# peleiden/librubiks

Hardware: AMD Instinct MI355X
Metric: cube node-expansions/sec (12-child fan-out) at 1M-state batch (higher is better)
Workload: dtype u8

## Files before the change

librubiks_amd/csrc/rk_cube_kernels.hip:

```cpp
#include <algorithm>
#include <atomic>
#include <cstdlib>
#include <mutex>
#include <vector>

#include "rk_device.h"
#include "rk_kernels.h"

namespace rk {

constexpr int EXP_ROUND = 64;
constexpr int EXP_WAVES = 4;
constexpr unsigned PACE_TAU_PS = 2100;
constexpr unsigned PACE_ROT_TAU_PS = 1200;
constexpr unsigned PACE_SOLVED_TAU_PS = 0;
constexpr unsigned PACE_LEAD_TICKS = 50;
constexpr unsigned PACE_PULL_WGS = 128;
constexpr unsigned PACE_PULL_WGS_FIRST = 256;
constexpr unsigned PACE_PHASE_TILES = 16384;
constexpr size_t PACE_MIN_TILES = 3072;
constexpr unsigned PACE686_MIN_PARENTS = 65536;
constexpr unsigned long long PACE_MAX_WAIT_TICKS = 2000;
constexpr unsigned long long PACE_STALE_TICKS = 1500;
constexpr size_t PACE_FIRST_TILES = 16384;
// ... 612 lines not shown
			#pragma unroll
			for (int k = 0; k < 20; k++) {
				const int idx = k * 64 + lane;
				buf_dw[idx] = idx < ndw ? got[k] : 0xFFFFFFFFu;
			}
		}
		wave_lds_fence();
		u32x4 v[5];
		#pragma unroll
		for (int k = 0; k < 5; k++) v[k] = buf[lane * 5 + k];
		const uint32_t s[20] = {v[0].x, v[0].y, v[0].z, v[0].w, v[1].x, v[1].y, v[1].z, v[1].w, v[2].x, v[2].y, v[2].z, v[2].w,
		                        v[3].x, v[3].y, v[3].z, v[3].w, v[4].x, v[4].y, v[4].z, v[4].w};
		uint32_t fl = 0;
		#pragma unroll
		for (int q = 0; q < 4; q++)
			if (4 * lane + q < np && is_solved5(&s[5 * q])) fl |= 1u << (8 * q);
		if (flags != nullptr) {
			uint8_t *fdst = flags + p0;
			if (np == ROW_TILE && ((reinterpret_cast<uintptr_t>(fdst) & 3) == 0)) {
				reinterpret_cast<uint32_t *>(fdst)[lane] = fl;
			} else {
				#pragma unroll
				for (int q = 0; q < 4; q++)
					if (4 * lane + q < np) fdst[4 * lane + q] = (uint8_t)((fl >> (8 * q)) & 1u);
			}
		}
		if (stats != nullptr && __ballot(fl != 0u) != 0ull && fl != 0u) {
			atomicAdd(reinterpret_cast<unsigned long long *>(&stats[0]), (unsigned long long)__popc(fl));
			const int firstq = (__ffs(fl) - 1) >> 3;
			atomicMin(&stats[1], (long long)(p0 + 4 * lane + firstq));
		}
		wave_lds_fence();
	}
}

template <int CH>
__device__ __forceinline__ void fetch_actions(const uint8_t *__restrict__ actions, size_t games, size_t g, int d0, int todo, uint32_t (&a)[CH])
{
	#pragma unroll
	for (int k = 0; k < CH; k++) a[k] = d0 + k < todo ? (uint32_t)actions[(size_t)(d0 + k) * games + g] : 0xFFu;
}

__global__ __launch_bounds__(256)
void k_apply_sequences(const uint8_t *__restrict__ actions, int moves, int games, int with_solved, int only_last,
                       uint32_t *__restrict__ out)
{
	__shared__ u32x4 s_act[36];
	stage_action_tables(s_act, threadIdx.x);
	__syncthreads();
	const int g = blockIdx.x * blockDim.x + threadIdx.x;
	if (g >= games) return;
	uint32_t s[5] = {SOLVED_DW[0], SOLVED_DW[1], SOLVED_DW[2], SOLVED_DW[3], SOLVED_DW[4]};
	const int rows = moves + (with_solved ? 1 : 0);
	uint32_t *o = out + (size_t)g * (only_last ? 1 : rows) * STATE_DWORDS;
	if (!only_last && with_solved) {
		#pragma unroll
		for (int j = 0; j < 5; j++) o[j] = s[j];
		o += STATE_DWORDS;
	}
	uint32_t worst = 0;
	constexpr int CH = 16;
	for (int d0 = 0; d0 < moves; d0 += CH) {
		uint32_t acts[CH];
		fetch_actions<CH>(actions, (size_t)games, (size_t)g, d0, moves, acts);
		#pragma unroll
		for (int k = 0; k < CH; k++) {
			if (d0 + k < moves) {
				uint32_t a = acts[k];
				worst = a > worst ? a : worst;
				a = a < 12u ? a : 0u;
				uint32_t tab[12];
				load_action_table(s_act, a, tab);
				move5(s, tab);
				if (!only_last) {
					#pragma unroll
					for (int j = 0; j < 5; j++) o[j] = s[j];
					o += STATE_DWORDS;
				}
			}
		}
	}
	if (only_last) {
		#pragma unroll
		for (int j = 0; j < 5; j++) o[j] = s[j];
	}
	if (worst >= 12u) atomicOr(&g_bad_actions, 1u);
}

__device__ __forceinline__ void scan_moves(uint32_t (&X)[12], int lane, int seg, int len)
{
	for (int off = 1; off < len; off <<= 1) {
		uint32_t Y[12];
		const int src = (lane - off) & 63;
		#pragma unroll
		for (int j = 0; j < 12; j++) Y[j] = (uint32_t)__builtin_amdgcn_ds_bpermute(src << 2, (int)X[j]);
		if (seg >= off) {
			uint32_t Z[12];
			#pragma unroll
			for (int j = 0; j < 6; j++) { Z[j] = lut4(Y[j], X); Z[6 + j] = lut4(Y[6 + j], X + 6); }
			#pragma unroll
			for (int j = 0; j < 12; j++) X[j] = Z[j];
		}
	}
}
__device__ __forceinline__ void identity_moves(uint32_t (&X)[12])
{
	#pragma unroll
	for (int j = 0; j < 6; j++) X[j] = X[6 + j] = 0x03020100u + 0x04040404u * (uint32_t)j;
}

__global__ __launch_bounds__(256)
void k_apply_sequences_scan(const uint8_t *__restrict__ actions, int moves, int games, int with_solved, int only_last, uint32_t *__restrict__ out)
{
	__shared__ u32x4 s_act[36];
	stage_action_tables(s_act, threadIdx.x);
	__syncthreads();
	const int lane = threadIdx.x & 63, g = blockIdx.x * 4 + (threadIdx.x >> 6);
	if (g >= games) return;
	uint32_t s[5] = {SOLVED_DW[0], SOLVED_DW[1], SOLVED_DW[2], SOLVED_DW[3], SOLVED_DW[4]};
	const int rows = moves + (with_solved ? 1 : 0);
	uint32_t *o = out + (size_t)g * (only_last ? 1 : rows) * STATE_DWORDS;
	if (!only_last && with_solved) {
		if (lane < 5) o[lane] = SOLVED_DW[lane];
		o += STATE_DWORDS;
	}
	uint32_t worst = 0;
	uint32_t a_next = lane < moves ? (uint32_t)actions[(size_t)lane * games + g] : 0xFFu;
	for (int d0 = 0; d0 < moves; d0 += 64) {
		const int n = moves - d0 < 64 ? moves - d0 : 64;
		uint32_t a = a_next;
		a_next = d0 + 64 + lane < moves ? (uint32_t)actions[(size_t)(d0 + 64 + lane) * games + g] : 0xFFu;
		uint32_t X[12];
		if (lane < n) {
			worst = a > worst ? a : worst;
			a = a < 12u ? a : 0u;
			load_action_table(s_act, a, X);
		} else {
			identity_moves(X);
		}
		scan_moves(X, lane, lane, n);
		uint32_t st[5] = {s[0], s[1], s[2], s[3], s[4]};
		move5(st, X);
		if (!only_last && lane < n) {
			#pragma unroll
			for (int j = 0; j < 5; j++) o[(size_t)(d0 + lane) * STATE_DWORDS + j] = st[j];
		}
		#pragma unroll
		for (int j = 0; j < 5; j++) s[j] = (uint32_t)__builtin_amdgcn_readlane((int)st[j], n - 1);
	}
	if (only_last && lane < 5) o[lane] = s[lane];
	if (worst >= 12u) atomicOr(&g_bad_actions, 1u);
}

__global__ __launch_bounds__(EXP_WAVES * WAVE)
void k_rollout_fanout(const uint8_t *__restrict__ actions, int moves, int games, int with_solved, uint32_t *__restrict__ states,
                      uint8_t *__restrict__ state_flags, u32x4 *__restrict__ children, uint32_t *__restrict__ solved, long long *__restrict__ stats)
{
	__shared__ u32x4 s_act[36];
	__shared__ u32x4 s_rows[48];
	__shared__ ExpandWaveLdsT<1> s_wave[EXP_WAVES];
	const int tid = threadIdx.x, lane = tid & 63, wv = tid >> 6;
	stage_action_tables(s_act, tid);
	if (tid < 48) {
		const uint32_t *src = reinterpret_cast<const uint32_t *>(D_TAB.rows) + 4 * tid;
		s_rows[tid] = u32x4{src[0], src[1], src[2], src[3]};
	}
	__syncthreads();
	const int rows = moves + (with_solved ? 1 : 0);
	const size_t n = (size_t)games * rows;
	const bool scan = rows <= EXP_ROUND;
	const int tile_states = scan ? (EXP_ROUND / rows) * rows : EXP_ROUND;
	const size_t p0 = ((size_t)blockIdx.x * EXP_WAVES + wv) * tile_states;
	if (p0 >= n) return;
	const int np = n - p0 < (size_t)tile_states ? (int)(n - p0) : tile_states;
	const size_t me = p0 + (lane < np ? lane : np - 1);
	const int g = (int)(me / rows), r = (int)(me - (size_t)g * rows);
	uint32_t par[5] = {SOLVED_DW[0], SOLVED_DW[1], SOLVED_DW[2], SOLVED_DW[3], SOLVED_DW[4]};
	uint32_t worst = 0;
	if (scan) {
		uint32_t X[12];
		const int mv = with_solved ? r - 1 : r;
		if (mv >= 0) {
			uint32_t a = actions[(size_t)mv * games + g];
			worst = a;
			a = a < 12u ? a : 0u;
			load_action_table(s_act, a, X);
		} else {
			identity_moves(X);
		}
		scan_moves(X, lane, r, rows);
		move5(par, X);
	} else {
		const int todo = with_solved ? r : r + 1;
		constexpr int CH = 16;
		for (int d0 = 0; d0 < todo; d0 += CH) {
			uint32_t acts[CH];
			fetch_actions<CH>(actions, (size_t)games, (size_t)g, d0, todo, acts);
			#pragma unroll
			for (int k = 0; k < CH; k++) {
				if (d0 + k < todo) {
					uint32_t a = acts[k];
					worst = a > worst ? a : worst;
					a = a < 12u ? a : 0u;
					uint32_t tab[12];
					load_action_table(s_act, a, tab);
					move5(par, tab);
				}
			}
		}
	}
	if (worst >= 12u) atomicOr(&g_bad_actions, 1u);
	const ExpandCtx c{s_rows, s_wave[wv].stage, s_wave[wv].flags, lane};
	uint32_t *stage_dw = reinterpret_cast<uint32_t *>(c.stage);
	#pragma unroll
	for (int j = 0; j < 5; j++) stage_dw[lane * 5 + j] = par[j];
	wave_lds_fence();
	#pragma unroll
	for (int k = 0; k < 5; k++) {
		const int idx = k * 64 + lane;
		if (idx < np * STATE_DWORDS) states[p0 * STATE_DWORDS + idx] = stage_dw[idx];
	}
	if (state_flags != nullptr && lane < np) state_flags[p0 + lane] = is_solved5(par) ? 1 : 0;
	wave_lds_fence();
	uint32_t out[60], fl[3];
	expand_lane<true>(c, par, out, fl);
	c.flags[lane * 3 + 0] = fl[0];
	c.flags[lane * 3 + 1] = fl[1];
	c.flags[lane * 3 + 2] = fl[2];
	#pragma unroll
	for (int v = 0; v < 15; v++)
		c.stage[lane * 15 + v] = u32x4{out[4 * v], out[4 * v + 1], out[4 * v + 2], out[4 * v + 3]};
	wave_lds_fence();
	u32x4 *dst = children + p0 * 15;
	const int nvec = np * 15;
	#pragma unroll
	for (int v = 0; v < 15; v++) {
		const int idx = v * 64 + lane;
		if (idx < nvec) store16<1>(dst, idx, c.stage[idx]);
	}
	uint32_t *fdst = solved + p0 * 3;
	#pragma unroll
	for (int k = 0; k < 3; k++) {
		const int idx = k * 64 + lane;
		if (idx < np * 3) fdst[idx] = c.flags[idx];
	}
	report_solved<true>(fl, lane < np, (p0 + lane) * 12, stats);
}

template <typename T> struct OhOne;
template <> struct OhOne<float>    { static constexpr uint32_t bits = 0x3F800000u; };
template <> struct OhOne<_Float16> { static constexpr uint32_t bits = 0x3C00u; };
struct bf16_tag {};
template <> struct OhOne<bf16_tag> { static constexpr uint32_t bits = 0x3F80u; };

template <typename T, int ELEM_BYTES, int TILE = 64, bool NT = false, int THREADS = 256>
__global__ __launch_bounds__(THREADS)
void k_as_oh(const uint32_t *__restrict__ states, u32x4 *__restrict__ out, size_t n, size_t n_tiles, unsigned tau_ps = 0, unsigned lead = 0,
             unsigned pull_wgs = 0, unsigned phase_tiles = 0, unsigned long long *pace = nullptr)
{
	constexpr int E = 16 / ELEM_BYTES;
	constexpr int CHUNKS_PER_ROW = 480 / E;
	constexpr int CHUNKS_PER_CUBIE = 24 / E;
	__shared__ uint32_t s_st[TILE * STATE_DWORDS];
	const int tid = threadIdx.x;
	const uint8_t *s_bytes = reinterpret_cast<const uint8_t *>(s_st);
	unsigned long long start = 0, base = 0;
	size_t tile_first = blockIdx.x, tile_stride = gridDim.x, slot = 0;
	if (tau_ps > 0) {
		const unsigned wgs_per_phase = pull_wgs + phase_tiles;
		const unsigned phase = blockIdx.x / wgs_per_phase, r = blockIdx.x - phase * wgs_per_phase;
		if (r < pull_wgs) {
			const size_t p_first = (size_t)phase * phase_tiles * TILE;
			const size_t p_count = n - p_first < (size_t)phase_tiles * TILE ? n - p_first : (size_t)phase_tiles * TILE;
			pull_front(states + p_first * STATE_DWORDS, p_count, (size_t)r * (THREADS / 64) + (tid >> 6), (size_t)pull_wgs * (THREADS / 64), tid & 63);
			if (tid == 0 && ((r & 63) == 63 || r + 1 == pull_wgs))
				__hip_atomic_fetch_max(pace, (unsigned long long)__builtin_amdgcn_s_memrealtime(), __ATOMIC_RELAXED, __HIP_MEMORY_SCOPE_AGENT);
			return;
		}
		start = __builtin_amdgcn_s_memrealtime();
		slot = r - pull_wgs;
		tile_first = (size_t)phase * phase_tiles + slot;
		tile_stride = n_tiles;
		if (pull_wgs == 0 && slot == 0 && tid == 0) __hip_atomic_fetch_max(pace, start, __ATOMIC_RELAXED, __HIP_MEMORY_SCOPE_AGENT);
		base = __hip_atomic_load(pace, __ATOMIC_RELAXED, __HIP_MEMORY_SCOPE_AGENT);
	}

	for (size_t tile = tile_first; tile < n_tiles; tile += tile_stride) {
		const size_t p0 = tile * TILE;
		const int np = (int)((n - p0 < (size_t)TILE) ? (n - p0) : (size_t)TILE);
		const int ndw = np * STATE_DWORDS;
		for (int idx = tid; idx < TILE * STATE_DWORDS; idx += THREADS) s_st[idx] = idx < ndw ? states[p0 * STATE_DWORDS + idx] : 0u;
		__syncthreads();
		PaceHold{base, start, slot, tau_ps, lead, tid & 63, pace}();
		const int nchunks = np * CHUNKS_PER_ROW;
		u32x4 *dst = out + p0 * CHUNKS_PER_ROW;
		for (int c = tid; c < nchunks; c += THREADS) {
			const int r = c / CHUNKS_PER_ROW, g = c - r * CHUNKS_PER_ROW;
			const int cubie = g / CHUNKS_PER_CUBIE;
			const int base = (g - cubie * CHUNKS_PER_CUBIE) * E;
			const int rel = (int)s_bytes[r * STATE_BYTES + cubie] - base;
			u32x4 val = {0u, 0u, 0u, 0u};
			if (ELEM_BYTES == 4) {
				val.x = rel == 0 ? OhOne<T>::bits : 0u;
				val.y = rel == 1 ? OhOne<T>::bits : 0u;
				val.z = rel == 2 ? OhOne<T>::bits : 0u;
				val.w = rel == 3 ? OhOne<T>::bits : 0u;
			} else {
				const uint32_t one = OhOne<T>::bits << (16 * (rel & 1));
				val.x = (rel >> 1) == 0 && rel >= 0 ? one : 0u;
				val.y = (rel >> 1) == 1 ? one : 0u;
				val.z = (rel >> 1) == 2 ? one : 0u;
				val.w = (rel >> 1) == 3 ? one : 0u;
			}
			if (NT) __builtin_nontemporal_store(val, dst + c);
			else dst[c] = val;
		}
		__syncthreads();
	}
}

__device__ __forceinline__ void stage_perm686(uint8_t *lds, int tid, int nthreads)
{
	const uint8_t *src = &D_TAB.perm686[0][0];
	for (int i = tid; i < N_ACTIONS * S686_SLOTS; i += nthreads) lds[i] = src[i];
}

template <bool FANOUT, bool FLAGS = false>
__global__ __launch_bounds__(256)
void k_rotate686(const uint16_t *__restrict__ states, const uint8_t *__restrict__ actions, u32x4 *__restrict__ out, size_t n_in,
                 uint8_t *__restrict__ flags = nullptr, long long *__restrict__ stats = nullptr)
{
	constexpr int GROUP = FANOUT ? 4 : 64;
	constexpr int OUT_PER_IN = FANOUT ? 12 : 1;
	__shared__ __attribute__((aligned(16))) uint8_t s_src[N_ACTIONS * 144];
	__shared__ __attribute__((aligned(16))) uint16_t s_in[GROUP * 144];
	__shared__ __attribute__((aligned(16))) uint8_t s_near[FLAGS ? N_ACTIONS * S686_SLOTS : 16];
	__shared__ __attribute__((aligned(16))) uint8_t s_col[FLAGS ? GROUP * S686_SLOTS : 16];
	if (threadIdx.x < N_ACTIONS * 144 / 16)
		reinterpret_cast<u32x4 *>(s_src)[threadIdx.x] = reinterpret_cast<const u32x4 *>(&D_TAB.src686[0][0])[threadIdx.x];
	if (FLAGS && threadIdx.x >= 128 && threadIdx.x < 128 + N_ACTIONS * S686_SLOTS / 16)
		reinterpret_cast<u32x4 *>(s_near)[threadIdx.x - 128] = reinterpret_cast<const u32x4 *>(&D_TAB.near686[0][0])[threadIdx.x - 128];
	const size_t n_groups = (n_in + GROUP - 1) / GROUP;
	constexpr int PW = (GROUP * 18 + 255) / 256;
	u32x4 pre[PW];
	const u32x4 *all4 = reinterpret_cast<const u32x4 *>(states);
	const size_t last_word = n_in * 18 - 1;
	auto request = [&](size_t group) {
		#pragma unroll
		for (int k = 0; k < PW; k++) {
			const size_t w = group * (GROUP * 18) + (size_t)(k * 256 + threadIdx.x);
			if (k * 256 + (int)threadIdx.x < GROUP * 18) pre[k] = all4[w < last_word ? w : last_word];
		}
	};
	if (blockIdx.x < n_groups) request(blockIdx.x);
	for (size_t g = blockIdx.x; g < n_groups; g += gridDim.x) {
		const size_t first = g * GROUP;
		const int ng = (int)((n_in - first < (size_t)GROUP) ? (n_in - first) : (size_t)GROUP);
		__syncthreads();
		#pragma unroll
		for (int k = 0; k < PW; k++) {
			const int i = k * 256 + threadIdx.x;
			if (i < GROUP * 18) reinterpret_cast<u32x4 *>(s_in)[i] = pre[k];
		}
		if (g + gridDim.x < n_groups) request(g + gridDim.x);
		__syncthreads();
		if (FLAGS && (int)threadIdx.x < ng * S686_SLOTS) {
			const uint16_t *h = s_in + threadIdx.x * 3;
			const uint32_t lo = (uint32_t)h[0] | ((uint32_t)h[1] << 16), hi = h[2];
			uint32_t col = 255u;
			if (hi == 0u) {
				if (lo == 0x00000001u) col = 0; else if (lo == 0x00000100u) col = 1;
				else if (lo == 0x00010000u) col = 2; else if (lo == 0x01000000u) col = 3;
			} else if (lo == 0u) {
				if (hi == 0x0001u) col = 4; else if (hi == 0x0100u) col = 5;
			}
			s_col[threadIdx.x] = (uint8_t)col;
		}
		u32x4 *dst = out + first * OUT_PER_IN * 18;
		const int n_chunks = ng * OUT_PER_IN * 18;
		for (int q = threadIdx.x; q < n_chunks; q += 256) {
			const int r = q / 18, k = q - r * 18;
			int local;
			uint32_t a;
			if (FANOUT) { local = r / 12; a = (uint32_t)(r - local * 12); }
			else        { local = r; a = actions[first + r]; if (a >= 12u) atomicOr(&g_bad_actions, 1u); a = a < 12u ? a : 0u; }
			const uint16_t *row = s_in + local * 144;
			const u32x2 offs = *reinterpret_cast<const u32x2 *>(&s_src[a * 144 + k * 8]);
			uint32_t h[8];
			#pragma unroll
			for (int i = 0; i < 8; i++) h[i] = row[((i < 4 ? offs.x : offs.y) >> (8 * (i & 3))) & 0xFFu];
			__builtin_nontemporal_store(u32x4{h[0] | (h[1] << 16), h[2] | (h[3] << 16), h[4] | (h[5] << 16), h[6] | (h[7] << 16)}, dst + q);
		}
		if (FLAGS) {
			__syncthreads();
			if ((int)threadIdx.x < ng * N_ACTIONS) {
				const int local = threadIdx.x / N_ACTIONS, a = threadIdx.x - local * N_ACTIONS;
				const uint32_t *c = reinterpret_cast<const uint32_t *>(s_col + local * S686_SLOTS);
				const uint32_t *w = reinterpret_cast<const uint32_t *>(s_near + a * S686_SLOTS);
				uint32_t diff = 0;
// ... 364 lines not shown
}

void launch_expand12(const int8_t *parents, int8_t *children, uint8_t *solved, long long *stats, size_t n, hipStream_t st)
{
	const size_t n_tiles = (n + EXP_ROUND - 1) / EXP_ROUND;
	const PaceConfig &pc = pace_config();
	if (n_tiles >= pc.min_tiles && pace_on(pc)) {
		const unsigned tau = fanout_tau(pc);
		if (tau != 0) { launch_expand12_paced(parents, children, solved, stats, n, pc, tau, st); return; }
	}
	launch_expand12_unpaced(parents, children, solved, stats, n, st);
}

int calibrate_pacing(bool force)
{
	PaceDevice *d = pace_device();
	if (d == nullptr) return -1;
	std::lock_guard<std::mutex> lk(d->cal_mu);
	if (d->source.load() != 0 && !force) return 0;
	const PaceConfig &pc = pace_config();
	auto settle = [&](int source, unsigned tau) { d->tau_ps.store(tau); d->source.store(source); return 0; };
	if (!pc.on || pc.tau_from_env || !pc.calibrate || pace_cells(d) == nullptr) return settle(2, pc.tau_ps);
	constexpr size_t N = (size_t)1 << 20;
	constexpr size_t B_PARENTS = N * STATE_BYTES, B_CHILDREN = 12 * N * STATE_BYTES, B_FLAGS = 12 * N;
	char *buf = nullptr;
	hipStream_t st = nullptr;
	hipEvent_t e0 = nullptr, e1 = nullptr;
	bool ok = hipMalloc((void **)&buf, B_PARENTS + B_CHILDREN + B_FLAGS + 256) == hipSuccess
	       && hipStreamCreateWithFlags(&st, hipStreamNonBlocking) == hipSuccess
	       && hipEventCreate(&e0) == hipSuccess && hipEventCreate(&e1) == hipSuccess;
	float best[PACE_CANDIDATES];
	for (float &b : best) b = 1e30f;
	if (ok) {
		int8_t *parents = (int8_t *)buf, *children = (int8_t *)(buf + B_PARENTS);
		uint8_t *flags = (uint8_t *)(buf + B_PARENTS + B_CHILDREN);
		long long *stats = (long long *)(buf + B_PARENTS + B_CHILDREN + B_FLAGS);
		ok = hipMemsetAsync(buf, 0, B_PARENTS, st) == hipSuccess && hipMemsetAsync(stats, 0, 16, st) == hipSuccess;
		(void)flags; (void)stats;
		auto go = [&](unsigned tau) {
			if (tau == 0) launch_expand12_unpaced(parents, children, nullptr, nullptr, N, st);
			else launch_expand12_paced(parents, children, nullptr, nullptr, N, pc, tau, st, false);
		};
		for (int round = 0; ok && round < 5; round++)
			for (int c = 0; ok && c < PACE_CANDIDATES; c++) {
				ok = hipEventRecord(e0, st) == hipSuccess;
				for (int k = 0; k < 4; k++) go(PACE_CANDIDATE_TAU_PS[c]);
				ok = ok && hipGetLastError() == hipSuccess && hipEventRecord(e1, st) == hipSuccess && hipEventSynchronize(e1) == hipSuccess;
				float ms = 0;
				ok = ok && hipEventElapsedTime(&ms, e0, e1) == hipSuccess;
				if (ok && round > 0 && ms * 250.0f < best[c]) best[c] = ms * 250.0f;
			}
	}
	if (e0) (void)hipEventDestroy(e0);
	if (e1) (void)hipEventDestroy(e1);
	if (st) (void)hipStreamDestroy(st);
	if (buf) (void)hipFree(buf);
	if (!ok) { (void)hipGetLastError(); return settle(2, pc.tau_ps); }
	int dflt = -1, win = 0;
	for (int c = 0; c < PACE_CANDIDATES; c++) {
		d->us[c] = best[c];
		if (PACE_CANDIDATE_TAU_PS[c] == pc.tau_ps) dflt = c;
		if (best[c] < best[win]) win = c;
	}
	if (dflt >= 0 && best[dflt] <= 1.03f * best[win]) win = dflt;
	return settle(1, PACE_CANDIDATE_TAU_PS[win]);
}

void get_pacing(unsigned *tau_ps, int *source, float *us)
{
	const PaceConfig &pc = pace_config();
	PaceDevice *d = pace_device();
	const int src = d ? d->source.load() : 0;
	if (tau_ps) *tau_ps = !pc.on ? 0u : (d && src == 1 ? d->tau_ps.load() : pc.tau_ps);
	if (source) *source = src;
	if (us) for (int c = 0; c < PACE_CANDIDATES; c++) us[c] = d ? d->us[c] : 0.0f;
}

void launch_expand12_soa(const uint32_t *parents, uint32_t *children, uint8_t *solved, long long *stats, size_t n, hipStream_t st)
{
	const unsigned grid = grid_for(n, 256, 1u << 20);
	if (solved != nullptr)
		hipLaunchKernelGGL(k_expand12_soa<true>, dim3(grid), dim3(256), 0, st, parents, children, solved, stats, n);
	else
		hipLaunchKernelGGL(k_expand12_soa<false>, dim3(grid), dim3(256), 0, st, parents, children, (uint8_t *)nullptr, (long long *)nullptr, n);
}

void launch_states_soa(const int8_t *states, uint32_t *planes, size_t n, bool to_soa, hipStream_t st)
{
	const unsigned grid = grid_for(n * 5, 256, 256u * 16u);
	hipLaunchKernelGGL(k_states_to_soa, dim3(grid), dim3(256), 0, st, (const uint32_t *)states, planes, n, to_soa ? 1 : 0);
}

static unsigned row_grid_cap()
{
	static const unsigned cap = [] { const char *e = std::getenv("RK_ROW_GRID"); return e ? (unsigned)std::atoi(e) : (1u << 22); }();
	return cap > 0 ? cap : (1u << 22);
}

static unsigned env_u(const char *name, unsigned dflt) { const char *e = std::getenv(name); return e ? (unsigned)std::atol(e) : dflt; }

void launch_multi_rotate(const int8_t *states, const uint8_t *actions, const uint8_t *dirs, int8_t *out, size_t n, hipStream_t st,
                         uint8_t *flags, long long *stats, bool with_flags)
{
	static const unsigned tau_cfg = env_u("RK_PACE_ROT_TAU_PS", PACE_ROT_TAU_PS), nt_cfg = env_u("RK_PACE_ROT_NT", 1);
	const size_t n_tiles = (n + ROW_TILE - 1) / ROW_TILE;
	const unsigned grid = grid_for(n_tiles, ROW_WAVES, row_grid_cap());
	const PaceConfig &pc = pace_config();
	const bool paced = pace_on(pc) && tau_cfg > 0 && n_tiles >= 8192 && (size_t)grid * ROW_WAVES >= n_tiles;
	const unsigned tau = paced ? tau_cfg : 0u, nt = paced ? nt_cfg : 0u;
	unsigned long long *const cell = paced ? next_pace_cell() : nullptr;
	PacedTurn turn(st, paced);
	if (with_flags)
		hipLaunchKernelGGL((k_multi_rotate<false, true>), dim3(grid), dim3(ROW_WAVES * WAVE), 0, st, (const uint32_t *)states, actions,
		                   (const uint8_t *)nullptr, (uint32_t *)out, n, n_tiles, tau, pc.lead, nt, cell, flags, stats);
	else if (dirs != nullptr)
		hipLaunchKernelGGL((k_multi_rotate<true, false>), dim3(grid), dim3(ROW_WAVES * WAVE), 0, st, (const uint32_t *)states, actions, dirs,
		                   (uint32_t *)out, n, n_tiles, tau, pc.lead, nt, cell, (uint8_t *)nullptr, (long long *)nullptr);
	else
		hipLaunchKernelGGL((k_multi_rotate<false, false>), dim3(grid), dim3(ROW_WAVES * WAVE), 0, st, (const uint32_t *)states, actions,
		                   (const uint8_t *)nullptr, (uint32_t *)out, n, n_tiles, tau, pc.lead, nt, cell, (uint8_t *)nullptr, (long long *)nullptr);
}

__global__ void k_take_bad_actions(unsigned *out) { if (threadIdx.x == 0 && blockIdx.x == 0) *out = atomicExch(&g_bad_actions, 0u); }

int read_bad_actions(hipStream_t st)
{
	unsigned *cell = nullptr;
	if (hipHostMalloc((void **)&cell, sizeof *cell, hipHostMallocDefault) != hipSuccess) return -1;
	*cell = 0;
	hipLaunchKernelGGL(k_take_bad_actions, dim3(1), dim3(64), 0, st, cell);
	const bool ok = hipGetLastError() == hipSuccess && hipStreamSynchronize(st) == hipSuccess;
	const unsigned h = *cell;
	(void)hipHostFree(cell);
	if (!ok) return -1;
	return h != 0 ? 1 : 0;
}

void launch_multi_is_solved(const int8_t *states, uint8_t *flags, long long *stats, size_t n, hipStream_t st)
{
	static const unsigned tau_cfg = env_u("RK_PACE_SOLVED_TAU_PS", PACE_SOLVED_TAU_PS);
	const size_t n_tiles = (n + ROW_TILE - 1) / ROW_TILE;
	const unsigned grid = grid_for(n_tiles, ROW_WAVES, row_grid_cap());
	const PaceConfig &pc = pace_config();
	const bool paced = pace_on(pc) && tau_cfg > 0 && n_tiles >= 8192 && (size_t)grid * ROW_WAVES >= n_tiles;
	PacedTurn turn(st, paced);
	hipLaunchKernelGGL(k_multi_is_solved, dim3(grid), dim3(ROW_WAVES * WAVE), 0, st, (const uint32_t *)states, flags, stats, n, n_tiles,
	                   paced ? tau_cfg : 0u, pc.lead, paced ? next_pace_cell() : (unsigned long long *)nullptr);
}

void launch_rollout_fanout(const uint8_t *actions, int moves, int games, int with_solved, int8_t *states, uint8_t *state_flags, int8_t *children,
                           uint8_t *child_flags, long long *stats, hipStream_t st)
{
	const size_t rows = (size_t)(moves + (with_solved ? 1 : 0)), n = (size_t)games * rows;
	const size_t tile_states = rows <= (size_t)EXP_ROUND ? (EXP_ROUND / rows) * rows : (size_t)EXP_ROUND;
	const unsigned grid = grid_for((n + tile_states - 1) / tile_states, EXP_WAVES, 1u << 22);
	hipLaunchKernelGGL(k_rollout_fanout, dim3(grid), dim3(EXP_WAVES * WAVE), 0, st, actions, moves, games, with_solved, (uint32_t *)states, state_flags,
	                   (u32x4 *)children, (uint32_t *)child_flags, stats);
}

void launch_apply_sequences(const uint8_t *actions, int moves, int games, int with_solved, int only_last, int8_t *out, hipStream_t st)
{
	if (games <= 1024 && moves >= 8) {
		hipLaunchKernelGGL(k_apply_sequences_scan, dim3(grid_for((size_t)games, 4, 1u << 22)), dim3(256), 0, st, actions, moves, games, with_solved, only_last, (uint32_t *)out);
		return;
	}
	const unsigned grid = grid_for((size_t)games, 256, 1u << 22);
	hipLaunchKernelGGL(k_apply_sequences, dim3(grid), dim3(256), 0, st, actions, moves, games, with_solved, only_last, (uint32_t *)out);
}

static unsigned oh_paced_grid(size_t n_tiles, unsigned pull, unsigned phase_tiles)
{
	const size_t n_phases = (n_tiles + phase_tiles - 1) / phase_tiles;
	return (unsigned)((n_phases - 1) * (size_t)(pull + phase_tiles) + pull + (n_tiles - (n_phases - 1) * phase_tiles));
}


void launch_as_oh(const int8_t *states, void *out, int out_dtype, size_t n, hipStream_t st)
{
	const PaceConfig &pc = pace_config();
	const size_t n_tiles = out_dtype == 0 ? (n + 7) / 8 : (n + 15) / 16;
	const bool paced = pace_on(pc) && n_tiles >= 8192;
	const unsigned tau = paced ? stream_tau(pc) * 15360u / 16128u : 0u;
	const unsigned phase_tiles = (unsigned)(((size_t)pc.phase_tiles * EXP_ROUND) / (out_dtype == 0 ? 8 : 16));
	const unsigned grid = paced ? oh_paced_grid(n_tiles, pc.pull_wgs, phase_tiles) : grid_for(n_tiles, 1, 1u << 22);
	PacedTurn turn(st, paced);
	#define RK_OH(T, EB, TL) do { \
		if (paced) hipLaunchKernelGGL((k_as_oh<T, EB, TL, true>), dim3(grid), dim3(256), 0, st, (const uint32_t *)states, (u32x4 *)out, n, n_tiles, tau, pc.lead, pc.pull_wgs, phase_tiles, next_pace_cell()); \
		else hipLaunchKernelGGL((k_as_oh<T, EB, TL, false>), dim3(grid), dim3(256), 0, st, (const uint32_t *)states, (u32x4 *)out, n, n_tiles, 0u, 0u, 0u, 0u, (unsigned long long *)nullptr); } while (0)
	if (out_dtype == 0) RK_OH(float, 4, 8);
	else if (out_dtype == 1) RK_OH(_Float16, 2, 16);
	else RK_OH(bf16_tag, 2, 16);
	#undef RK_OH
}

void launch_rotate686(const int8_t *states, const uint8_t *actions, int8_t *out, size_t n_out, bool fanout, hipStream_t st,
                      uint8_t *flags, long long *stats)
{
	if (fanout) {
		const size_t n_in = n_out / 12;
		{
			static const unsigned min_parents = env_u("RK_PACE686_MIN", PACE686_MIN_PARENTS);
			const PaceConfig &pc = pace_config();
			if (pace_on(pc) && n_in >= min_parents) {
				constexpr unsigned G = 8;
				const size_t n_groups = (n_in + G - 1) / G;
				const unsigned phase_groups = (unsigned)(((size_t)pc.phase_tiles * 4) / G);
				const unsigned tau = (unsigned)((unsigned long long)stream_tau(pc) * (G * 12 * S686_BYTES + G * 12) / 16128u);
				const size_t n_phases = (n_groups + phase_groups - 1) / phase_groups;
				const unsigned grid = (unsigned)((n_phases - 1) * (size_t)(pc.pull_wgs + phase_groups) + pc.pull_wgs + (n_groups - (n_phases - 1) * phase_groups));
				PacedTurn turn(st, true);
				if (flags != nullptr || stats != nullptr)
					hipLaunchKernelGGL((k_fanout686p<true, G>), dim3(grid), dim3(256), 0, st, (const uint16_t *)states, (u32x4 *)out, n_in, flags, stats,
					                   pc.pull_wgs, phase_groups, tau, pc.lead, next_pace_cell());
				else
					hipLaunchKernelGGL((k_fanout686p<false, G>), dim3(grid), dim3(256), 0, st, (const uint16_t *)states, (u32x4 *)out, n_in, (uint8_t *)nullptr,
					                   (long long *)nullptr, pc.pull_wgs, phase_groups, tau, pc.lead, next_pace_cell());
				return;
			}
		}
		const unsigned grid = grid_for(n_in, 4, 8192u);
		if (flags != nullptr || stats != nullptr)
			hipLaunchKernelGGL((k_rotate686<true, true>), dim3(grid), dim3(256), 0, st, (const uint16_t *)states, actions, (u32x4 *)out, n_in, flags, stats);
		else
			hipLaunchKernelGGL((k_rotate686<true, false>), dim3(grid), dim3(256), 0, st, (const uint16_t *)states, actions, (u32x4 *)out, n_in,
			                   (uint8_t *)nullptr, (long long *)nullptr);
	} else {
		const unsigned grid = grid_for(n_out, 64, 2048u);
		hipLaunchKernelGGL((k_rotate686<false, false>), dim3(grid), dim3(256), 0, st, (const uint16_t *)states, actions, (u32x4 *)out, n_out,
		                   (uint8_t *)nullptr, (long long *)nullptr);
	}
}

void launch_is_solved686(const int8_t *states, uint8_t *flags, long long *stats, size_t n, hipStream_t st)
{
	const unsigned grid = grid_for(n, 128, 1u << 20);
	hipLaunchKernelGGL(k_is_solved686, dim3(grid), dim3(256), 0, st, (const u32x4 *)states, flags, stats, n);
}

void launch_as_oh686(const int8_t *states, void *out, int out_dtype, size_t n, hipStream_t st)
{
	const size_t ndw = n * 72;
	const unsigned grid = grid_for(ndw, 256, 256u * 8u);
	if (out_dtype == 0)
		hipLaunchKernelGGL((k_as_oh686<float, 4>), dim3(grid), dim3(256), 0, st, (const uint32_t *)states, (u32x4 *)out, ndw);
	else if (out_dtype == 1)
		hipLaunchKernelGGL((k_as_oh686<_Float16, 2>), dim3(grid), dim3(256), 0, st, (const uint32_t *)states, (u32x4 *)out, ndw);
	else
		hipLaunchKernelGGL((k_as_oh686<bf16_tag, 2>), dim3(grid), dim3(256), 0, st, (const uint32_t *)states, (u32x4 *)out, ndw);
}

void launch_as_correct686(const int8_t *states, float *out, size_t n, hipStream_t st)
{
	const unsigned grid = grid_for(n * 48, 256, 256u * 8u);
	hipLaunchKernelGGL(k_as_correct686, dim3(grid), dim3(256), 0, st, states, out, n * 48);
}

const Tables &host_tables()
{
	static const Tables t = make_tables();
	return t;
}

}
```

Before: 24.91 billion.

## Use full 64-state tiles with prefix walk and persistent multi-tile waves in rollout fanout

The rollout fanout kernel now tiles states in fixed 64-state blocks that can cross game boundaries, instead of rounding tiles down to whole games. Each tile reconstructs the state of the partial game at its start with a lane-parallel prefix walk over earlier moves. Each wave loops over several tiles in a grid-stride pattern and prefetches the next tile's actions. Full tiles use an unmasked emit path with vectorized flag stores. The aim is to fill every lane and amortize LDS table staging across tiles, at the cost of a serial prefix walk per tile and more complex indexing.

```diff
diff --git a/librubiks_amd/csrc/rk_cube_kernels.hip b/librubiks_amd/csrc/rk_cube_kernels.hip
--- a/librubiks_amd/csrc/rk_cube_kernels.hip
+++ b/librubiks_amd/csrc/rk_cube_kernels.hip
@@ -788,65 +788,16 @@
 	if (worst >= 12u) atomicOr(&g_bad_actions, 1u);
 }
 
-__global__ __launch_bounds__(EXP_WAVES * WAVE)
-void k_rollout_fanout(const uint8_t *__restrict__ actions, int moves, int games, int with_solved, uint32_t *__restrict__ states,
-                      uint8_t *__restrict__ state_flags, u32x4 *__restrict__ children, uint32_t *__restrict__ solved, long long *__restrict__ stats)
-{
-	__shared__ u32x4 s_act[36];
-	__shared__ u32x4 s_rows[48];
-	__shared__ ExpandWaveLdsT<1> s_wave[EXP_WAVES];
-	const int tid = threadIdx.x, lane = tid & 63, wv = tid >> 6;
-	stage_action_tables(s_act, tid);
-	if (tid < 48) {
-		const uint32_t *src = reinterpret_cast<const uint32_t *>(D_TAB.rows) + 4 * tid;
-		s_rows[tid] = u32x4{src[0], src[1], src[2], src[3]};
-	}
-	__syncthreads();
-	const int rows = moves + (with_solved ? 1 : 0);
-	const size_t n = (size_t)games * rows;
-	const bool scan = rows <= EXP_ROUND;
-	const int tile_states = scan ? (EXP_ROUND / rows) * rows : EXP_ROUND;
-	const size_t p0 = ((size_t)blockIdx.x * EXP_WAVES + wv) * tile_states;
-	if (p0 >= n) return;
-	const int np = n - p0 < (size_t)tile_states ? (int)(n - p0) : tile_states;
-	const size_t me = p0 + (lane < np ? lane : np - 1);
-	const int g = (int)(me / rows), r = (int)(me - (size_t)g * rows);
-	uint32_t par[5] = {SOLVED_DW[0], SOLVED_DW[1], SOLVED_DW[2], SOLVED_DW[3], SOLVED_DW[4]};
-	uint32_t worst = 0;
-	if (scan) {
-		uint32_t X[12];
-		const int mv = with_solved ? r - 1 : r;
-		if (mv >= 0) {
-			uint32_t a = actions[(size_t)mv * games + g];
-			worst = a;
-			a = a < 12u ? a : 0u;
-			load_action_table(s_act, a, X);
-		} else {
-			identity_moves(X);
-		}
-		scan_moves(X, lane, r, rows);
-		move5(par, X);
-	} else {
-		const int todo = with_solved ? r : r + 1;
-		constexpr int CH = 16;
-		for (int d0 = 0; d0 < todo; d0 += CH) {
-			uint32_t acts[CH];
-			fetch_actions<CH>(actions, (size_t)games, (size_t)g, d0, todo, acts);
-			#pragma unroll
-			for (int k = 0; k < CH; k++) {
-				if (d0 + k < todo) {
-					uint32_t a = acts[k];
-					worst = a > worst ? a : worst;
-					a = a < 12u ? a : 0u;
-					uint32_t tab[12];
-					load_action_table(s_act, a, tab);
-					move5(par, tab);
-				}
-			}
-		}
-	}
-	if (worst >= 12u) atomicOr(&g_bad_actions, 1u);
-	const ExpandCtx c{s_rows, s_wave[wv].stage, s_wave[wv].flags, lane};
+constexpr unsigned RF_RESIDENT_WAVES = 2048;
+constexpr unsigned RF_TILES_PER_WAVE = 2;
+constexpr int RF_PREFIX_WALK = 1;
+
+template <bool FULL>
+__device__ __forceinline__ void rollout_emit(const ExpandCtx &c, const uint32_t par[5], size_t p0, int np, uint32_t *__restrict__ states,
+                                             uint8_t *__restrict__ state_flags, u32x4 *__restrict__ children, uint32_t *__restrict__ solved,
+                                             long long *__restrict__ stats)
+{
+	const int lane = c.lane;
 	uint32_t *stage_dw = reinterpret_cast<uint32_t *>(c.stage);
 	#pragma unroll
 	for (int j = 0; j < 5; j++) stage_dw[lane * 5 + j] = par[j];
@@ -854,9 +805,9 @@
 	#pragma unroll
 	for (int k = 0; k < 5; k++) {
 		const int idx = k * 64 + lane;
-		if (idx < np * STATE_DWORDS) states[p0 * STATE_DWORDS + idx] = stage_dw[idx];
-	}
-	if (state_flags != nullptr && lane < np) state_flags[p0 + lane] = is_solved5(par) ? 1 : 0;
+		if (FULL || idx < np * STATE_DWORDS) states[p0 * STATE_DWORDS + idx] = stage_dw[idx];
+	}
+	if (state_flags != nullptr && (FULL || lane < np)) state_flags[p0 + lane] = is_solved5(par) ? 1 : 0;
 	wave_lds_fence();
 	uint32_t out[60], fl[3];
 	expand_lane<true>(c, par, out, fl);
@@ -872,15 +823,142 @@
 	#pragma unroll
 	for (int v = 0; v < 15; v++) {
 		const int idx = v * 64 + lane;
-		if (idx < nvec) store16<1>(dst, idx, c.stage[idx]);
+		if (FULL || idx < nvec) store16<1>(dst, idx, c.stage[idx]);
 	}
 	uint32_t *fdst = solved + p0 * 3;
-	#pragma unroll
-	for (int k = 0; k < 3; k++) {
-		const int idx = k * 64 + lane;
-		if (idx < np * 3) fdst[idx] = c.flags[idx];
-	}
-	report_solved<true>(fl, lane < np, (p0 + lane) * 12, stats);
+	if (FULL && (reinterpret_cast<uintptr_t>(fdst) & 15) == 0) {
+		if (lane < 48) store16<1>(reinterpret_cast<u32x4 *>(fdst), lane, reinterpret_cast<const u32x4 *>(c.flags)[lane]);
+	} else {
+		#pragma unroll
+		for (int k = 0; k < 3; k++) {
+			const int idx = k * 64 + lane;
+			if (FULL || idx < np * 3) fdst[idx] = c.flags[idx];
+		}
+	}
+	report_solved<true>(fl, FULL || lane < np, (p0 + lane) * 12, stats);
+	wave_lds_fence();
+}
+
+template <int PREFIX_WALK>
+__global__ __launch_bounds__(EXP_WAVES * WAVE)
+void k_rollout_fanout(const uint8_t *__restrict__ actions, int moves, int games, int with_solved, uint32_t *__restrict__ states,
+                      uint8_t *__restrict__ state_flags, u32x4 *__restrict__ children, uint32_t *__restrict__ solved, long long *__restrict__ stats)
+{
+	__shared__ u32x4 s_act[36];
+	__shared__ u32x4 s_rows[48];
+	__shared__ ExpandWaveLdsT<1> s_wave[EXP_WAVES];
+	const int tid = threadIdx.x, lane = tid & 63, wv = tid >> 6;
+	const uint32_t rows = (uint32_t)(moves + (with_solved ? 1 : 0));
+	const size_t n = (size_t)games * rows;
+	const uint32_t n_tiles = (uint32_t)((n + EXP_ROUND - 1) / EXP_ROUND);
+	const uint32_t first = __builtin_amdgcn_readfirstlane(blockIdx.x * EXP_WAVES + wv), stride = gridDim.x * EXP_WAVES;
+	const bool scan = rows <= (uint32_t)EXP_ROUND;
+
+	auto coords = [&](uint32_t t, uint32_t &g0, uint32_t &r0, uint32_t &g, uint32_t &r, int &np) {
+		const uint32_t p0 = t * EXP_ROUND;
+		np = n - p0 < (size_t)EXP_ROUND ? (int)(n - p0) : EXP_ROUND;
+		g0 = p0 / rows; r0 = p0 - g0 * rows;
+		const uint32_t tt = r0 + (uint32_t)(lane < np ? lane : np - 1);
+		const uint32_t q = tt / rows;
+		g = g0 + q; r = tt - q * rows;
+	};
+	auto fetch = [&](uint32_t t, uint32_t &own, uint32_t &pre) {
+		uint32_t g0, r0, g, r; int np;
+		coords(t, g0, r0, g, r, np);
+		const int mv = (int)r - with_solved, pmv = lane - with_solved;
+		own = mv >= 0 ? (uint32_t)actions[(size_t)mv * games + g] : 0u;
+		pre = ((uint32_t)lane < r0 && pmv >= 0) ? (uint32_t)actions[(size_t)pmv * games + g0] : 0u;
+	};
+
+	uint32_t a_own = 0, a_pre = 0;
+	if (scan && first < n_tiles) fetch(first, a_own, a_pre);
+	stage_action_tables(s_act, tid);
+	if (tid < 48) {
+		const uint32_t *src = reinterpret_cast<const uint32_t *>(D_TAB.rows) + 4 * tid;
+		s_rows[tid] = u32x4{src[0], src[1], src[2], src[3]};
+	}
+	__syncthreads();
+	const ExpandCtx c{s_rows, s_wave[wv].stage, s_wave[wv].flags, lane};
+	uint32_t worst = 0;
+
+	for (uint32_t t = first; t < n_tiles; t += stride) {
+		uint32_t g0, r0, g, r; int np;
+		coords(t, g0, r0, g, r, np);
+		uint32_t par[5] = {SOLVED_DW[0], SOLVED_DW[1], SOLVED_DW[2], SOLVED_DW[3], SOLVED_DW[4]};
+		if (scan) {
+			worst = a_own > worst ? a_own : worst;
+			worst = a_pre > worst ? a_pre : worst;
+			uint32_t X[12];
+			if ((int)r - with_solved >= 0) load_action_table(s_act, a_own < 12u ? a_own : 0u, X);
+			else identity_moves(X);
+			if (r0 > 0) {
+				uint32_t s0[5];
+				if (PREFIX_WALK) {
+					uint32_t s = lane == 0 ? SOLVED_DW[0] : lane == 1 ? SOLVED_DW[1] : lane == 2 ? SOLVED_DW[2] : lane == 3 ? SOLVED_DW[3] : SOLVED_DW[4];
+					const uint32_t *half = reinterpret_cast<const uint32_t *>(s_act) + (lane >= 2 ? 6 : 0);
+					auto table_of_row = [&](uint32_t j, uint32_t (&tb)[6]) {
+						uint32_t a = (uint32_t)__builtin_amdgcn_readlane((int)a_pre, (int)j);
+						a = a < 12u ? a : 0u;
+						#pragma unroll
+						for (int k = 0; k < 6; k++) tb[k] = half[a * 12 + k];
+					};
+					uint32_t j = (uint32_t)with_solved;
+					uint32_t tb[6];
+					if (j < r0) table_of_row(j, tb);
+					for (; j < r0; j++) {
+						uint32_t nb[6] = {0, 0, 0, 0, 0, 0};
+						if (j + 1 < r0) table_of_row(j + 1, nb);
+						s = lut4(s, tb);
+						#pragma unroll
+						for (int k = 0; k < 6; k++) tb[k] = nb[k];
+					}
+					#pragma unroll
+					for (int k = 0; k < 5; k++) s0[k] = (uint32_t)__builtin_amdgcn_readlane((int)s, k);
+				} else {
+					uint32_t P[12];
+					if ((uint32_t)lane < r0 && lane - with_solved >= 0) load_action_table(s_act, a_pre < 12u ? a_pre : 0u, P);
+					else identity_moves(P);
+					scan_moves(P, lane, lane, (int)r0);
+					uint32_t pre[12];
+					#pragma unroll
+					for (int k = 0; k < 12; k++) pre[k] = (uint32_t)__builtin_amdgcn_readlane((int)P[k], (int)r0 - 1);
+					#pragma unroll
+					for (int k = 0; k < 5; k++) s0[k] = SOLVED_DW[k];
+					move5(s0, pre);
+				}
+				if ((uint32_t)lane + r0 < rows) {
+					#pragma unroll
+					for (int k = 0; k < 5; k++) par[k] = s0[k];
+				}
+			}
+			scan_moves(X, lane, (int)r < lane ? (int)r : lane, (int)rows);
+			move5(par, X);
+			const uint32_t tn = t + stride;
+			if (tn < n_tiles) fetch(tn, a_own, a_pre);
+		} else {
+			const int todo = with_solved ? (int)r : (int)r + 1;
+			constexpr int CH = 16;
+			for (int d0 = 0; d0 < todo; d0 += CH) {
+				uint32_t acts[CH];
+				fetch_actions<CH>(actions, (size_t)games, (size_t)g, d0, todo, acts);
+				#pragma unroll
+				for (int k = 0; k < CH; k++) {
+					if (d0 + k < todo) {
+						uint32_t a = acts[k];
+						worst = a > worst ? a : worst;
+						a = a < 12u ? a : 0u;
+						uint32_t tab[12];
+						load_action_table(s_act, a, tab);
+						move5(par, tab);
+					}
+				}
+			}
+		}
+		const size_t p0 = (size_t)t * EXP_ROUND;
+		if (np == EXP_ROUND) rollout_emit<true>(c, par, p0, np, states, state_flags, children, solved, stats);
+		else rollout_emit<false>(c, par, p0, np, states, state_flags, children, solved, stats);
+	}
+	if (worst >= 12u) atomicOr(&g_bad_actions, 1u);
 }
 
 template <typename T> struct OhOne;
@@ -1551,10 +1629,22 @@
                            uint8_t *child_flags, long long *stats, hipStream_t st)
 {
 	const size_t rows = (size_t)(moves + (with_solved ? 1 : 0)), n = (size_t)games * rows;
-	const size_t tile_states = rows <= (size_t)EXP_ROUND ? (EXP_ROUND / rows) * rows : (size_t)EXP_ROUND;
-	const unsigned grid = grid_for((n + tile_states - 1) / tile_states, EXP_WAVES, 1u << 22);
-	hipLaunchKernelGGL(k_rollout_fanout, dim3(grid), dim3(EXP_WAVES * WAVE), 0, st, actions, moves, games, with_solved, (uint32_t *)states, state_flags,
-	                   (u32x4 *)children, (uint32_t *)child_flags, stats);
+	const size_t n_tiles = (n + EXP_ROUND - 1) / EXP_ROUND;
+	unsigned per_wave = n_tiles < RF_RESIDENT_WAVES ? 1u : RF_TILES_PER_WAVE;
+	int walk = RF_PREFIX_WALK;
+#ifdef RK_TUNING
+	const unsigned k_cfg = env_u("RK_RF_TILES_PER_WAVE", 0), grid_cfg = env_u("RK_RF_GRID", 0), walk_cfg = env_u("RK_RF_PREFIX_WALK", RF_PREFIX_WALK);
+	if (k_cfg > 0) per_wave = k_cfg;
+	walk = (int)walk_cfg;
+#endif
+	unsigned grid = grid_for(n_tiles, (size_t)EXP_WAVES * per_wave, 1u << 22);
+#ifdef RK_TUNING
+	if (grid_cfg > 0) grid = grid_cfg;
+#endif
+	if (walk) hipLaunchKernelGGL(k_rollout_fanout<1>, dim3(grid), dim3(EXP_WAVES * WAVE), 0, st, actions, moves, games, with_solved, (uint32_t *)states, state_flags,
+	                             (u32x4 *)children, (uint32_t *)child_flags, stats);
+	else hipLaunchKernelGGL(k_rollout_fanout<0>, dim3(grid), dim3(EXP_WAVES * WAVE), 0, st, actions, moves, games, with_solved, (uint32_t *)states, state_flags,
+	                        (u32x4 *)children, (uint32_t *)child_flags, stats);
 }
 
 void launch_apply_sequences(const uint8_t *actions, int moves, int games, int with_solved, int only_last, int8_t *out, hipStream_t st)
```

Measured after the change: 24.94 billion, median of 2. Within noise of the previous version (+0.1%).
